# microsoft/crescent-credentials

Measured on AMD Instinct MI355X. Metric: Groth16 proofs/sec (rs256-sd-shaped circuit, BN254), G1 MSM scalar-adds/sec reported alongside, higher is better.
Workload: dtype u32 limbs (BN254 Fq/Fr, 254-bit modular integers)

## Files before the change

crescent-credentials_amd/csrc/msm.hip:

```cpp
#include "msm.hpp"
#include "g2pair.hpp"

#include <chrono>
#include <cstring>
#include <type_traits>

namespace cg {

static constexpr int SCALAR_BITS = 255;

int msm_default_window(uint64_t n, bool precomputed) {
    double best = 1e300;
    int best_c = 4;
    for (int c = 4; c <= 22; ++c) {
        int W = (SCALAR_BITS + c - 1) / c;
        if ((double)W * (double)n >= 2147483648.0) continue;
        double buckets = (double)(1u << (c - 1)) * (precomputed ? 1 : W);
        if (buckets > (double)(1u << 24)) continue;
        double cost = (double)n * W * 12.0 + buckets * 2.0 * 16.0;
        if (cost < best) { best = cost; best_c = c; }
    }
    return best_c;
}

// ... 950 lines not shown
                XYZZ29<F29T> Cu = shfl_up_acc(Cv, d);
                const bool Cuinf = __shfl_up((int)Cinf, d, 64) != 0;
                const bool fu = __shfl_up((int)f, d, 64) != 0;
                if (f) add29(Cv, Cinf, Cu, Cuinf);
                f = f && fu;
            }
        }
        XYZZ29<F29T> Pv = shfl_up_acc(Cv, 1);
        const bool Pinf = __shfl_up((int)Cinf, 1, 64) != 0;
        const unsigned long long chain = __ballot(single && (lane == 0 || joinL));
        auto open_left = [&](unsigned j) { return (~chain & (j >= 63 ? ~0ull : ((2ull << j) - 1ull))) == 0ull; };
        auto emit = [&](uint32_t key, const XYZZ29<F29T>& v, bool vinf, bool touches_left) {
            if (key == NO_KEY) return;
            if (touches_left && !final_level) {
                out_keys[2 * wv] = key;
                store_acc(out_pts + (size_t)(2 * wv) * ACC, v, vinf);
            } else {
                store_acc(bucket_sums + (size_t)key * ACC, v, vinf);
            }
        };
        if (lane > 0 && !joinL) emit(kPrev, Pv, Pinf, open_left(lane - 1));
        if (!single) {
            XYZZ29<F29T> H = A;
            bool Hinf = Ainf, left = lane == 0;
            if (joinL) { add29(H, Hinf, Pv, Pinf); left = open_left(lane - 1); }
            emit(kF, H, Hinf, left);
        }
        if (lane == 63) {
            if (final_level) {
                emit(kL, Cv, Cinf, false);
            } else if (open_left(63)) {
                emit(kL, Cv, Cinf, true);
                out_keys[2 * wv + 1] = kL;
                store_acc(out_pts + (size_t)(2 * wv + 1) * ACC, Cv, true);
            } else {
                out_keys[2 * wv + 1] = kL;
                store_acc(out_pts + (size_t)(2 * wv + 1) * ACC, Cv, Cinf);
            }
        }
    }
}

template <class F29T>
__device__ __forceinline__ void block_tree_sum(XYZZ29<F29T>& acc, bool& inf, uint32_t* sm) {
    constexpr int ACC = Words29<F29T>::ACC;
    store_acc(sm + (size_t)threadIdx.x * ACC, acc, inf);
    __syncthreads();
    for (uint32_t s = blockDim.x / 2; s > 0; s >>= 1) {
        if (threadIdx.x < s) {
            XYZZ29<F29T> b;
            bool bi = load_acc(sm + (size_t)(threadIdx.x + s) * ACC, b);
            add29(acc, inf, b, bi);
            store_acc(sm + (size_t)threadIdx.x * ACC, acc, inf);
        }
        __syncthreads();
    }
}

template <class F29T>
__global__ void __launch_bounds__(256) k_bucket_rows_cols(const uint32_t* __restrict__ buckets, uint32_t R, uint32_t C,
                                                          uint32_t* __restrict__ rows, uint32_t* __restrict__ cols) {
    constexpr int ACC = Words29<F29T>::ACC;
    extern __shared__ __attribute__((aligned(16))) uint32_t sm[];
    const uint32_t w = blockIdx.y, b = blockIdx.x;
    const bool is_row = b < R;
    const uint32_t count = is_row ? C : R, base = is_row ? b * C : b - R, stride = is_row ? 1u : C;
    const uint32_t* src = buckets + (size_t)w * R * C * ACC;
    XYZZ29<F29T> acc;
    bool inf = true;
    for (uint32_t k = threadIdx.x; k < count; k += blockDim.x) {
        XYZZ29<F29T> q;
        bool qinf = load_acc(src + ((size_t)base + (size_t)k * stride) * ACC, q);
        add29(acc, inf, q, qinf);
    }
    block_tree_sum(acc, inf, sm);
    if (threadIdx.x == 0) {
        uint32_t* dst = is_row ? rows + ((size_t)w * R + b) * ACC : cols + ((size_t)w * C + (b - R)) * ACC;
        store_acc(dst, acc, inf);
    }
}

static constexpr uint32_t RED_CHUNK = 32;
template <class F29T>
__global__ void __launch_bounds__(256) k_bucket_chunks(uint32_t* __restrict__ buckets, uint32_t R, uint32_t C,
                                                      uint32_t* __restrict__ rowp, uint32_t* __restrict__ colp, int zero_after) {
    constexpr int ACC = Words29<F29T>::ACC;
    const uint32_t w = blockIdx.y;
    const uint32_t KC = (C + RED_CHUNK - 1) / RED_CHUNK, KR = (R + RED_CHUNK - 1) / RED_CHUNK;
    const uint32_t tile = blockIdx.x * (blockDim.x >> 6) + (threadIdx.x >> 6);
    if (tile >= KR * KC) return;
    const uint32_t tr = tile / KC, tc = tile - tr * KC;
    const uint32_t lane = threadIdx.x & 63u, i = lane & 31u;
    const bool row_lane = lane < 32u;
    uint32_t* src = buckets + (size_t)w * R * C * ACC;
    const uint32_t r0 = tr * RED_CHUNK, c0 = tc * RED_CHUNK;
    const uint32_t nr = R - r0 < RED_CHUNK ? R - r0 : RED_CHUNK, nc = C - c0 < RED_CHUNK ? C - c0 : RED_CHUNK;
    XYZZ29<F29T> acc;
    bool inf = true;
    const bool live = row_lane ? i < nr : i < nc;
    const uint32_t steps = row_lane ? nc : nr;
    for (uint32_t s = 0; s < RED_CHUNK; ++s) {
        if (live && s < steps) {
            const uint32_t r = row_lane ? r0 + i : r0 + s, col = row_lane ? c0 + s : c0 + i;
            XYZZ29<F29T> q;
            bool qinf = load_acc(src + ((size_t)r * C + col) * ACC, q);
            add29(acc, inf, q, qinf);
        }
    }
    if (live) {
        if (row_lane) store_acc(rowp + ((size_t)w * R * KC + (size_t)(r0 + i) * KC + tc) * ACC, acc, inf);
        else store_acc(colp + ((size_t)w * KR * C + (size_t)tr * C + (c0 + i)) * ACC, acc, inf);
    }
    if (zero_after) {
        static_assert(ACC % 4 == 0, "accumulator records are whole uint4s");
        const uint32_t row_vecs = nc * (ACC / 4);
        for (uint32_t r = 0; r < nr; ++r) {
            uint4* dst = reinterpret_cast<uint4*>(src + ((size_t)(r0 + r) * C + c0) * ACC);
            for (uint32_t k = lane; k < row_vecs; k += 64u) dst[k] = make_uint4(0u, 0u, 0u, 0u);
        }
    }
}
template <class F29T>
__global__ void __launch_bounds__(256) k_bucket_chunk_sums(const uint32_t* __restrict__ rowp, const uint32_t* __restrict__ colp, uint32_t R,
                                                          uint32_t C, uint32_t* __restrict__ rows, uint32_t* __restrict__ cols) {
    constexpr int ACC = Words29<F29T>::ACC;
    const uint32_t w = blockIdx.y;
    const uint32_t KC = (C + RED_CHUNK - 1) / RED_CHUNK, KR = (R + RED_CHUNK - 1) / RED_CHUNK;
    const uint32_t n_row = (R + 63u) & ~63u;
    const uint32_t t = blockIdx.x * blockDim.x + threadIdx.x;
    XYZZ29<F29T> acc;
    bool inf = true;
    if (t < n_row) {
        if (t >= R) return;
        const uint32_t* src = rowp + ((size_t)w * R + t) * KC * ACC;
        for (uint32_t k = 0; k < KC; ++k) {
            XYZZ29<F29T> q;
            bool qinf = load_acc(src + (size_t)k * ACC, q);
            add29(acc, inf, q, qinf);
        }
        store_acc(rows + ((size_t)w * R + t) * ACC, acc, inf);
    } else {
        const uint32_t col = t - n_row;
        if (col >= C) return;
        const uint32_t* src = colp + (size_t)w * KR * C * ACC;
        for (uint32_t k = 0; k < KR; ++k) {
            XYZZ29<F29T> q;
            bool qinf = load_acc(src + ((size_t)k * C + col) * ACC, q);
            add29(acc, inf, q, qinf);
        }
        store_acc(cols + ((size_t)w * C + col) * ACC, acc, inf);
    }
}

template <class F29T>
__global__ void __launch_bounds__(256) k_bit_sums(const uint32_t* __restrict__ rows, uint32_t R, uint32_t rbits,
                                                  const uint32_t* __restrict__ cols, uint32_t C, uint32_t* __restrict__ out,
                                                  uint32_t* plan, uint32_t* __restrict__ plan_out, uint32_t zero_words) {
    constexpr int ACC = Words29<F29T>::ACC;
    extern __shared__ __attribute__((aligned(16))) uint32_t sm[];
    const uint32_t w = blockIdx.y, b = blockIdx.x;
    if (w == 0 && b == 0 && threadIdx.x < PLAN_WORDS) {
        plan_out[threadIdx.x] = plan[threadIdx.x];
        if (zero_words) plan[threadIdx.x] = 0;
    }
    if (zero_words) {
        const uint32_t nthr = gridDim.x * gridDim.y * blockDim.x, me = (w * gridDim.x + b) * blockDim.x + threadIdx.x;
        for (uint32_t k = PLAN_WORDS + me; k < zero_words; k += nthr) plan[k] = 0;
    }
    const bool is_row = b < rbits;
    const uint32_t bit = is_row ? b : b - rbits, n = is_row ? R : C, offset = is_row ? 0u : 1u;
    const uint32_t* src = is_row ? rows + (size_t)w * R * ACC : cols + (size_t)w * C * ACC;
    XYZZ29<F29T> acc;
    bool inf = true;
    for (uint32_t i = threadIdx.x; i < n; i += blockDim.x) {
        if (((i + offset) >> bit) & 1u) {
            XYZZ29<F29T> q;
            bool qinf = load_acc(src + (size_t)i * ACC, q);
            add29(acc, inf, q, qinf);
        }
    }
    block_tree_sum(acc, inf, sm);
    if (threadIdx.x == 0) store_acc(out + ((size_t)w * gridDim.x + b) * ACC, acc, inf);
}

static constexpr uint32_t ACC_TARGET_THREADS = 256u * 4u * 4u * 64u;
static constexpr uint32_t G2PAIR_RESIDENT_WAVES = 2;
static constexpr uint32_t ACC_TARGET_PAIRS = 256u * 4u * G2PAIR_RESIDENT_WAVES * 64u / 2u;
template <class F29T> static uint32_t acc_target_segments(bool latency_mode) {
    static const uint32_t quarters = [] { const char* e = CG_TUNE_ENV("ACC_QUARTERS"); const int v = e ? atoi(e) : 4; return (uint32_t)(v >= 1 && v <= 16 ? v : 4); }();
    const uint32_t full = latency_mode ? ACC_TARGET_THREADS : ACC_TARGET_THREADS / 4u * quarters;
    if (Words29<F29T>::NF != 2) return full;
    return g2_pair_kernel(latency_mode) ? ACC_TARGET_PAIRS : full;
}
static constexpr uint32_t ACC_MIN_L = 64, ACC_MIN_L_LATENCY = 16;
static constexpr uint32_t ACC_LEVEL_L = 8;

static int red_cbits(int c) { return (c - 1 + 1) / 2 > 10 ? 10 : (c - 1 + 1) / 2; }

static void part_bits(int c, int W, bool precomputed, int& bits1, int& bits2) {
    int key_bits = c - 1;
    if (!precomputed) key_bits += ilog2_ceil((uint64_t)W);
    if (key_bits < 1) key_bits = 1;
    if (key_bits <= PART_MAX_BITS) { bits1 = key_bits; bits2 = 0; return; }
    bits1 = (key_bits + 1) / 2;
    if (const char* e = CG_TUNE_ENV("PART_BITS1_DELTA")) {
        const int b = bits1 + atoi(e);
        if (b >= 1 && b <= PART_MAX_BITS && key_bits - b >= 1 && key_bits - b <= PART_MAX_BITS) bits1 = b;
    }
    bits2 = key_bits - bits1;
}

template <class F>
void MsmEngine<F>::init(const MsmBases<F>* b, hipStream_t zero_stream) {
    bases = b;
    const uint64_t n = b->n;
    const int W = b->W;
    cap_entries = n * (uint64_t)W;
    if (cap_entries == 0) cap_entries = 1;
    const uint32_t nb = 1u << (b->c - 1);
    nbuckets_total = b->precomputed ? nb : nb * (uint32_t)W;
    part_bits(b->c, W, b->precomputed, bits1, bits2);
    if (bits1 > PART_MAX_BITS || bits2 > PART_MAX_BITS) throw HipError(CG_ERR_INVALID_ARGUMENT, "bucket key space too large");
    const uint32_t B1 = 1u << bits1;
    const uint64_t tiles = n ? ceil_div(n, PART_TILE) : 1;
    blk_hist.alloc(tiles * B1);
    const size_t keyspace = bits2 ? ((size_t)1 << (bits1 + bits2)) : 0;
    counters.alloc(PLAN_WORDS + 2 * (size_t)B1 * PART_PAD + 2 * keyspace);
    starts.alloc(2 * ((size_t)B1 + 1) + 2);
    max_chunks = bits2 ? (uint32_t)(cap_entries / PART_CHUNK) + B1 + 1 : 0;
    bucket_sums.alloc(((size_t)nbuckets_total + 1) * ACC);
    min_L = latency_mode ? ACC_MIN_L_LATENCY : ACC_MIN_L;
    if (const char* e = CG_TUNE_ENV("MIN_SEGMENT")) {
        const int v = atoi(e);
        if (v >= 1 && v <= 4096) min_L = (uint32_t)v;
    }
    uint64_t t1 = (cap_entries + min_L - 1) / min_L;
    if (t1 > acc_target_segments<F29T>(latency_mode)) t1 = acc_target_segments<F29T>(latency_mode);
    max_segments = (uint32_t)t1;
    uint64_t pa = 2 * t1, pb = 0;
    for (uint64_t w = ceil_div(t1, 64); ; w = ceil_div(w, 64)) { pb += 2 * w; if (w <= 1) break; }
    mem().reserve(cap_entries, bits2 ? cap_entries : 1, pa, pa * ACC, pb, pb * ACC);
    const uint32_t wins = b->precomputed ? 1u : (uint32_t)W;
    {
        const int cbits = red_cbits(b->c);
        const uint32_t C = 1u << cbits, R = nb / C;
        red_rbits = ilog2_ceil((uint64_t)R);
        red_cbits1 = cbits + 1;
        rows_buf.alloc((size_t)R * wins * ACC);
        cols_buf.alloc((size_t)C * wins * ACC);
        if (!latency_mode) {
            rowp_buf.alloc((size_t)R * ceil_div(C, RED_CHUNK) * wins * ACC);
            colp_buf.alloc((size_t)ceil_div(R, RED_CHUNK) * C * wins * ACC);
        }
    }
    if (zero_stream) {
        CG_HIP(hipMemsetAsync(counters.p, 0, counters.bytes(), zero_stream));
        CG_HIP(hipMemsetAsync(bucket_sums.p, 0, bucket_sums.bytes(), zero_stream));
    } else {
        hipStream_t zs = nullptr;
        CG_HIP(hipStreamCreateWithFlags(&zs, hipStreamNonBlocking));
        hipError_t e1 = hipMemsetAsync(counters.p, 0, counters.bytes(), zs);
        hipError_t e2 = hipMemsetAsync(bucket_sums.p, 0, bucket_sums.bytes(), zs);
        hipError_t e3 = hipStreamSynchronize(zs);
        (void)hipStreamDestroy(zs);
        CG_HIP(e1); CG_HIP(e2); CG_HIP(e3);
// ... 8 lines not shown

template <class F>
void MsmEngine<F>::device_bytes(uint64_t& entries, uint64_t& pieces, uint64_t& other) const {
    entries += own_mem.entry_bytes();
    pieces += own_mem.piece_bytes();
    other += blk_hist.bytes() + counters.bytes() + starts.bytes() + bucket_sums.bytes() + rows_buf.bytes() + cols_buf.bytes() +
             rowp_buf.bytes() + colp_buf.bytes();
}

static float elapsed_ms(hipEvent_t a, hipEvent_t b) {
    float ms = 0;
    if (hipEventElapsedTime(&ms, a, b) != hipSuccess) return 0.f;
    return ms;
}
template <class F> float MsmEngine<F>::ms_total() const { return elapsed_ms(ev_t[0], ev_t[5]); }
template <class F> float MsmEngine<F>::ms_sort() const { return n_scalars ? elapsed_ms(ev_t[1], ev_t[2]) : 0.f; }
template <class F> float MsmEngine<F>::ms_accum() const { return n_scalars ? elapsed_ms(ev_t[3], ev_t[4]) : 0.f; }

template <class F>
MsmEngine<F>::~MsmEngine() {
    for (auto& e : ev_t) if (e) (void)hipEventDestroy(e);
}

template <class F>
void MsmEngine<F>::digits(const Fr* scalars_dev, uint64_t n, hipStream_t st) {
    if (n > bases->n) n = bases->n;
    n_scalars = n;
    adopted = nullptr;
    for (int k = 0; k < PLAN_WORDS; ++k) h_plan.p[k] = 0;
    CG_HIP(hipEventRecord(ev_t[0], st));
    if (!n) {
        if (!counters_clean) fill_zero(counters.p, (counters.bytes() + 15) & ~(size_t)15, st);
        counters_clean = zero_at_end;
        return;
    }
    const uint32_t B1 = 1u << bits1;
    uint32_t* plan = counters.p;
    uint32_t* hist1 = plan + PLAN_WORDS;
    uint32_t* cur1 = hist1 + (size_t)B1 * PART_PAD;
    uint32_t* hist2 = cur1 + (size_t)B1 * PART_PAD;
    uint32_t* cur2 = hist2 + (bits2 ? ((size_t)1 << (bits1 + bits2)) : 0);
    uint32_t* start1 = starts.p;
    uint32_t* chunk0 = starts.p + B1 + 1;
    PartShape sh;
    sh.n = (uint32_t)n; sh.c = bases->c; sh.W = bases->W; sh.precomputed = bases->precomputed ? 1 : 0;
    sh.row_stride = (uint32_t)bases->n;
    sh.bits1 = bits1; sh.bits2 = bits2;
    sh.staged = latency_mode ? 1 : 0;
    const uint32_t tiles = ceil_div(n, PART_TILE);
    CG_HIP(hipEventRecord(ev_t[1], st));
    if (!counters_clean) fill_zero(counters.p, (counters.bytes() + 15) & ~(size_t)15, st);
    counters_clean = false;
    PlanArgs pa;
    pa.start1 = start1; pa.chunk0 = chunk0; pa.target_threads = acc_target_segments<F29T>(latency_mode); pa.min_L = min_L;
    pa.two_level = bits2 ? 1 : 0;
    launch_part_level1(true, sh, tiles, (size_t)B1 * 4, st, scalars_dev, bases->valid.p, blk_hist.p, hist1, plan, nullptr, nullptr, nullptr, pa);
    CG_KERNEL_CHECK();
    launch_part_level1(false, sh, tiles, (size_t)B1 * 4, st, scalars_dev, bases->valid.p, blk_hist.p, nullptr, nullptr, start1, cur1, mem().ent_a.p, pa);
    CG_KERNEL_CHECK();
    if (bits2) {
        const uint32_t B2 = 1u << bits2;
        k_part_count2<<<max_chunks, 256, (size_t)B2 * 4, st>>>(bits1, bits2, mem().ent_a.p, chunk0, start1, hist2);
        CG_KERNEL_CHECK();
        k_part_place2<<<max_chunks, 256, (size_t)B2 * 16 + (size_t)PART_CHUNK * 8, st>>>(bits1, bits2, mem().ent_a.p, chunk0, start1, hist2, cur2, mem().ent_b.p);
        CG_KERNEL_CHECK();
    }
    CG_HIP(hipEventRecord(ev_t[2], st));
}

template <class F>
void MsmEngine<F>::adopt(const uint64_t* grouped_entries, const uint32_t* plan_dev, uint64_t n, hipStream_t st) {
    if (n > bases->n) n = bases->n;
    n_scalars = n;
    for (int k = 0; k < PLAN_WORDS; ++k) h_plan.p[k] = 0;
    CG_HIP(hipEventRecord(ev_t[0], st));
    CG_HIP(hipEventRecord(ev_t[1], st));
    k_replan<<<1, 1, 0, st>>>(counters.p, plan_dev, acc_target_segments<F29T>(latency_mode), min_L);
    counters_clean = false;
    CG_KERNEL_CHECK();
    CG_HIP(hipEventRecord(ev_t[2], st));
    adopted = n ? grouped_entries : nullptr;
}

template <class F>
void MsmEngine<F>::accumulate(hipStream_t st) {
    if (!buckets_clean) fill_zero(bucket_sums.p, bucket_sums.bytes(), st);
    buckets_clean = false;
    if (n_scalars) {
        const uint32_t* plan = counters.p;
        const uint64_t* grouped = adopted ? adopted : this->grouped();
        CG_HIP(hipEventRecord(ev_t[3], st));
        static const bool knock_accum = CG_TUNE_ENV("KNOCK_ACCUM") != nullptr, knock_combine = CG_TUNE_ENV("KNOCK_COMBINE") != nullptr;
        if (!knock_accum)
            launch_accum_affine<F29T>(grouped, plan, max_segments, bases->table.p, bucket_sums.p, mem().part_keys_a.p, mem().part_pts_a.p, latency_mode, st);
        CG_KERNEL_CHECK();
        CG_HIP(hipEventRecord(ev_t[4], st));
        if (max_segments > 1 && !knock_accum && !knock_combine) {
            MsmScratch& S = mem();
            uint32_t segs = max_segments;
            for (int level = 0; segs > 1; ++level) {
                const uint32_t waves = ceil_div(segs, 64u);
                k_combine_wave<F29T><<<ceil_div(waves, tail_block<F29T>() / 64u), tail_block<F29T>(), 0, st>>>(S.part_keys_a.p, S.part_pts_a.p, plan, bucket_sums.p, S.part_keys_b.p, S.part_pts_b.p, level);
                CG_KERNEL_CHECK();
                segs = waves;
            }
        }
    }
    enqueue_reduction(st);
    CG_HIP(hipEventRecord(ev_t[5], st));
}

template <class F>
void MsmEngine<F>::enqueue_reduction(hipStream_t st) {
    const uint32_t wins = bases->precomputed ? 1u : (uint32_t)bases->W;
    const uint32_t nb = 1u << (bases->c - 1);
    const uint32_t C = 1u << red_cbits(bases->c), R = nb / C;
    const size_t lds = (size_t)256 * ACC * 4;
    static const bool force_tree = CG_TUNE_ENV("RED_TREE") != nullptr;
    static const bool knock_tail = CG_TUNE_ENV("KNOCK_TAIL") != nullptr;
    if (knock_tail) return;
    if (latency_mode || force_tree) {
        k_bucket_rows_cols<F29T><<<dim3(R + C, wins), 256, lds, st>>>(bucket_sums.p, R, C, rows_buf.p, cols_buf.p);
        CG_KERNEL_CHECK();
    } else {
        const uint32_t KC = ceil_div(C, RED_CHUNK), KR = ceil_div(R, RED_CHUNK);
        const uint32_t lanes_b = ((R + 63u) & ~63u) + C;
        const uint32_t tb = tail_block<F29T>();
        k_bucket_chunks<F29T><<<dim3(ceil_div(KR * KC, tb / 64u), wins), tb, 0, st>>>(bucket_sums.p, R, C, rowp_buf.p, colp_buf.p, zero_at_end ? 1 : 0);
        CG_KERNEL_CHECK();
        buckets_clean = zero_at_end;
        k_bucket_chunk_sums<F29T><<<dim3(ceil_div(lanes_b, tb), wins), tb, 0, st>>>(rowp_buf.p, colp_buf.p, R, C, rows_buf.p, cols_buf.p);
        CG_KERNEL_CHECK();
    }
    const uint32_t nbits = (uint32_t)(red_rbits + red_cbits1);
    k_bit_sums<F29T><<<dim3(nbits, wins), 256, lds, st>>>(rows_buf.p, R, (uint32_t)red_rbits, cols_buf.p, C, h_result.dev(), counters.p,
                                                          h_plan.dev(), zero_at_end ? (uint32_t)counters.n : 0u);
    CG_KERNEL_CHECK();
    counters_clean = zero_at_end;
}

static Fq fq_from_limbs29(const uint32_t l[9]) {
    typedef unsigned __int128 u128;
    uint64_t v[5] = {0, 0, 0, 0, 0};
    for (int i = 0; i < 9; ++i) {
        int bit = 29 * i, w = bit >> 6, sh = bit & 63;
        u128 x = (u128)l[i] << sh;
        u128 s = (u128)v[w] + (uint64_t)x;
        v[w] = (uint64_t)s;
        u128 carry = (s >> 64) + (x >> 64);
        for (int k = w + 1; k < 5 && carry; ++k) {
            u128 t = (u128)v[k] + (uint64_t)carry;
            v[k] = (uint64_t)t;
            carry = t >> 64;
        }
    }
    uint64_t n[5] = {0, 0, 0, 0, 0};
    for (int i = 0; i < 4; ++i) n[i] = (uint64_t)FqP::N[2 * i] | ((uint64_t)FqP::N[2 * i + 1] << 32);
    auto ge = [&]() {
        for (int i = 4; i >= 0; --i) {
            if (v[i] > n[i]) return true;
            if (v[i] < n[i]) return false;
        }
        return true;
    };
    while (ge()) {
        u128 br = 0;
        for (int i = 0; i < 5; ++i) {
            u128 d = (u128)v[i] - n[i] - (uint64_t)br;
            v[i] = (uint64_t)d;
            br = (d >> 64) & 1;
        }
    }
    Fq a;
    for (int i = 0; i < 4; ++i) { a.l[2 * i] = (uint32_t)v[i]; a.l[2 * i + 1] = (uint32_t)(v[i] >> 32); }
    Fq c2 = Fq::zero();
    c2.l[7] = 0x08000000u;
    return mul(a, c2);
}
static void coord_from_limbs29(Fq& out, const uint32_t* w) { out = fq_from_limbs29(w); }
static void coord_from_limbs29(Fq2& out, const uint32_t* w) { out.c0 = fq_from_limbs29(w); out.c1 = fq_from_limbs29(w + 9); }

template <class F>
static XYZZ<F> xyzz_from_words(const uint32_t* w, int acc_words) {
    const int q = acc_words / 4;
    bool inf = true;
    for (int i = 0; i < q; ++i) if (w[2 * q + i]) inf = false;
    if (inf) return XYZZ<F>::inf();
    XYZZ<F> r;
    coord_from_limbs29(r.x, w);
    coord_from_limbs29(r.y, w + q);
    coord_from_limbs29(r.zz, w + 2 * q);
    coord_from_limbs29(r.zzz, w + 3 * q);
    return r;
}

template <class F>
static XYZZ<F> fold_bits(const uint32_t* bit_sums, int n, int acc_words) {
    XYZZ<F> acc = XYZZ<F>::inf();
    for (int k = n - 1; k >= 0; --k) {
        acc = dbl(acc);
        add(acc, xyzz_from_words<F>(bit_sums + (size_t)k * acc_words, acc_words));
    }
    return acc;
}
template <class F>
static XYZZ<F> window_value(const uint32_t* bit_sums, int acc_words, int rbits, int cbits1) {
    XYZZ<F> rows = fold_bits<F>(bit_sums, rbits, acc_words);
    XYZZ<F> cols = fold_bits<F>(bit_sums + (size_t)rbits * acc_words, cbits1, acc_words);
    for (int k = 0; k < cbits1 - 1; ++k) rows = dbl(rows);
    add(rows, cols);
    return rows;
}

template <class F>
XYZZ<F> MsmEngine<F>::value() const {
    const int nbits = red_rbits + red_cbits1;
    if (bases->precomputed) return window_value<F>(h_result.p, ACC, red_rbits, red_cbits1);
    const int W = bases->W, c = bases->c;
    XYZZ<F> acc = XYZZ<F>::inf();
    for (int j = W - 1; j >= 0; --j) {
        for (int k = 0; k < c; ++k) acc = dbl(acc);
// ... 115 lines not shown
```

crescent-credentials_amd/csrc/msm.hpp:

```cpp
#pragma once
#include "common.hpp"
#include "curve29.hpp"
#include "ntt.hpp"

#include <functional>

namespace cg {

template <class F>
struct MsmBases {
    typedef typename To29<F>::type F29T;
    static constexpr int AFF = Words29<F29T>::AFF;
    uint64_t n = 0;
    int c = 0;
    int W = 0;
    bool precomputed = true;
    DevBuf<uint32_t> table;
    DevBuf<uint8_t> valid;
    void build(const Affine<F>* bases_dev, uint64_t n, int c, bool precompute, hipStream_t st);
    void build_from_row0(const uint32_t* row0_dev, const uint8_t* valid_dev, uint64_t n, int c, hipStream_t st);
    int rebuild(int c_new, hipStream_t st);
    void alloc_rows(uint64_t n, int c, bool precompute);
    void expand_rows(hipStream_t st);
};

int msm_default_window(uint64_t n, bool precomputed);
int msm_best_window(uint64_t n_bases, double nz_small, double nz_full);

struct MsmScratch {
    DevBuf<uint64_t> ent_a, ent_b;
    DevBuf<uint32_t> part_keys_a, part_keys_b;
    DevBuf<uint32_t> part_pts_a, part_pts_b;
    uint64_t entry_bytes() const { return ent_a.bytes() + ent_b.bytes(); }
    uint64_t piece_bytes() const { return part_keys_a.bytes() + part_keys_b.bytes() + part_pts_a.bytes() + part_pts_b.bytes(); }
    void reserve(size_t n_ent_a, size_t n_ent_b, size_t keys_a, size_t pts_a, size_t keys_b, size_t pts_b) {
        if (ent_a.n < n_ent_a) ent_a.alloc(n_ent_a);
        if (ent_b.n < n_ent_b) ent_b.alloc(n_ent_b);
        if (part_keys_a.n < keys_a) part_keys_a.alloc(keys_a);
        if (part_pts_a.n < pts_a) part_pts_a.alloc(pts_a);
        if (part_keys_b.n < keys_b) part_keys_b.alloc(keys_b);
        if (part_pts_b.n < pts_b) part_pts_b.alloc(pts_b);
    }
};

template <class F>
struct MsmEngine {
    typedef typename To29<F>::type F29T;
    static constexpr int ACC = Words29<F29T>::ACC;
    const MsmBases<F>* bases = nullptr;
    uint64_t cap_entries = 0;
    uint32_t nbuckets_total = 0;
    MsmScratch own_mem;
    MsmScratch* shared_mem = nullptr;
    MsmScratch& mem() { return shared_mem ? *shared_mem : own_mem; }
    const MsmScratch& mem() const { return shared_mem ? *shared_mem : own_mem; }
    int bits1 = 0, bits2 = 0;
    DevBuf<uint32_t> blk_hist;
    DevBuf<uint32_t> counters;
    DevBuf<uint32_t> starts;
    uint32_t max_chunks = 0;
    uint32_t min_L = 16;
    uint32_t max_segments = 0;
    DevBuf<uint32_t> bucket_sums;
    DevBuf<uint32_t> rows_buf, cols_buf;
    DevBuf<uint32_t> rowp_buf, colp_buf;
    int red_rbits = 0, red_cbits1 = 0;
    PinnedBuf<uint32_t> h_plan;
    PinnedBuf<uint32_t> h_result;
    uint64_t n_scalars = 0;
    bool zero_at_end = false;
    bool counters_clean = false, buckets_clean = false;
    bool latency_mode = false;
    uint32_t n_entries() const { return h_plan.p ? h_plan.p[0] : 0; }
    uint32_t n_nonzero() const { return h_plan.p ? h_plan.p[3] : 0; }
    void enqueue_reduction(hipStream_t st);
    hipEvent_t ev_t[6] = {nullptr, nullptr, nullptr, nullptr, nullptr, nullptr};
    float ms_total() const;
    float ms_sort() const;
    float ms_accum() const;

    void init(const MsmBases<F>* b, hipStream_t zero_stream = nullptr);
    ~MsmEngine();
    void device_bytes(uint64_t& entries, uint64_t& pieces, uint64_t& other) const;
    void digits(const Fr* scalars_dev, uint64_t n, hipStream_t st);
    template <class G>
    bool can_adopt(const MsmEngine<G>& src) const {
        return bases->precomputed && src.bases->precomputed && bases->n == src.bases->n && bases->c == src.bases->c &&
               bits1 == src.bits1 && bits2 == src.bits2;
    }
    void adopt(const uint64_t* grouped_entries, const uint32_t* plan_dev, uint64_t n, hipStream_t st);
    const uint64_t* grouped() const { return bits2 ? mem().ent_b.p : mem().ent_a.p; }
    const uint64_t* adopted = nullptr;
    void accumulate(hipStream_t st);
    XYZZ<F> value() const;
};

void ec_inverse_dft(const uint32_t* row0_in, const uint8_t* valid_in, uint64_t n_in, int logn, const Fr& scale_base,
                    const Fr& scale_mult, uint32_t* row0_out, uint8_t* valid_out, hipStream_t st);
void ec_transform_h_bases(const uint32_t* row0_in, const uint8_t* valid_in, uint64_t n_in, int logn, uint32_t* row0_out,
                          uint8_t* valid_out, hipStream_t st);
void ec_fold_c_into_l(const uint32_t* h_row0, const uint8_t* h_valid, uint64_t n_h, int logn, const Fr& vanishing_inv,
                      const cg_csr& c_matrix, uint64_t num_constraints, uint64_t num_inputs, uint64_t M,
                      const uint32_t* l_row0, const uint8_t* l_valid, uint32_t* row0_out, uint8_t* valid_out, hipStream_t st);
void ec_fold_ct_into_l(const uint32_t* h_row0, const uint8_t* h_valid, uint64_t n_h, int logn, const Fr& vanishing_inv,
                       const HostCsc& c_transposed, uint64_t num_constraints, uint64_t num_inputs, uint64_t M,
                       const uint32_t* l_row0, const uint8_t* l_valid, uint32_t* row0_out, uint8_t* valid_out, hipStream_t st);
void sum_xyzz_by_key(const uint32_t* keys, const uint32_t* pts, uint64_t count, uint32_t* sums, hipStream_t st);
void build_hl_bases_folded(MsmBases<Fq>& out_h, MsmBases<Fq>& out_l, const Affine<Fq>* h_bases_dev, uint64_t n_h, int logn,
                           const Affine<Fq>* l_bases_dev, uint64_t num_inputs, uint64_t M, const cg_csr& c_matrix,
                           uint64_t num_constraints, const Fr& vanishing_inv, uint64_t h_first, uint64_t h_stride, uint64_t h_count,
                           int c_h, uint64_t l_first, uint64_t l_count, int c_l, hipStream_t st, float* ms_fold = nullptr,
                           float* ms_tables = nullptr);

void build_h_bases_folded(MsmBases<Fq>& out_h, const uint32_t* h_row0, const uint8_t* h_valid, uint64_t n_h, int logn, uint64_t h_first,
                          uint64_t h_stride, uint64_t h_count, int c_h, hipStream_t st, float* ms_fold, float* ms_tables);
void build_l_bases_folded(MsmBases<Fq>& out_l, const uint32_t* h_row0, const uint8_t* h_valid, uint64_t n_h, int logn,
                          const uint32_t* l_row0, const uint8_t* l_valid, uint64_t num_inputs, uint64_t M, const HostCsc& c_transposed,
                          uint64_t num_constraints, const Fr& vanishing_inv, uint64_t l_first, uint64_t l_count,
                          const std::function<int()>& pick_c_l, hipStream_t st, float* ms_fold, float* ms_tables);

template <class F>
void import_bases(const uint8_t* host_bytes, uint32_t coord_form, uint64_t n, Affine<F>* out_dev, hipStream_t st);

extern template struct MsmBases<Fq>;
extern template struct MsmBases<Fq2>;
extern template struct MsmEngine<Fq>;
extern template struct MsmEngine<Fq2>;

}
```

crescent-credentials_amd/csrc/prover.hip:

```cpp
#include <atomic>
#include <condition_variable>
#include <shared_mutex>
#include <memory>
#include <mutex>
#include <chrono>
#include <cstdlib>
#include <exception>
#include <functional>
#include <thread>

#include "msm.hpp"
#include "ntt.hpp"
#include "wmap29.hpp"

namespace cg {

const char* csr_view_problem(const cg_csr& m);

std::string& last_error() {
    static thread_local std::string e;
    return e;
}
int fail(int code, const char* fmt, ...) {
    char buf[1024];
// ... 919 lines not shown
    for (int i = 0; i < 5; ++i)
        if (i == 0 || S->st[i] != S->st[0]) CG_HIP(hipEventSynchronize(S->ev_fin[i]));
}

static float upload_assignment(cg_ctx* c, Upload* u, const void* host_assignment, bool timed) {
    if (timed) CG_HIP(hipEventRecord(u->ev[0], u->st));
    CG_HIP(hipMemcpyAsync(u->w.p, host_assignment, c->M * 32, hipMemcpyHostToDevice, u->st));
    if (timed) CG_HIP(hipEventRecord(u->ev[1], u->st));
    if (c->spin_wait || c->latency) {
        CG_HIP(hipStreamSynchronize(u->st));
    } else {
        CG_HIP(hipEventRecord(u->ev_done, u->st));
        wait_sleeping(u->ev_done, 50);
    }
    return timed ? ev_ms(u->ev[0], u->ev[1]) : 0.f;
}

static const char* const BROKEN_CONTEXT = "a window re-tune ran out of device memory while re-sizing the proof slots: free this context and load the circuit again";

struct CallFrame {
    CallGuard inside;
    cg_ctx* const c;
    const Fr* w_dev = nullptr;
    ProofSlot* S = nullptr;
    float upload_ms = 0.f;
    CallFrame(cg_ctx* ctx, const void* assignment, bool on_device, bool may_run_alone, bool timed = false, bool handle = false)
        : inside(ctx), c(ctx), in_handle(handle), exceptions(std::uncaught_exceptions()) {
        try {
            if (c->broken) throw HipError(CG_ERR_OUT_OF_MEMORY, BROKEN_CONTEXT);
            CG_HIP(hipSetDevice(c->device));
            if (in_handle) c->tune_mu.lock_shared_passing_waiting_writers();
            else c->tune_mu.lock_shared();
            gate_held = true;
            if (c->broken) throw HipError(CG_ERR_OUT_OF_MEMORY, BROKEN_CONTEXT);
            w_dev = (const Fr*)assignment;
            if (!on_device) {
                up = c->acquire_upload();
                upload_ms = upload_assignment(c, up, assignment, timed);
                w_dev = up->w.p;
            }
            S = c->acquire(may_run_alone);
        } catch (...) {
            release();
            throw;
        }
    }
    ~CallFrame() { release(); }
    void release() {
        if (S) {
            if (in_handle || std::uncaught_exceptions() > exceptions)
                for (auto st : S->st) if (st) (void)hipStreamSynchronize(st);
            c->release(S);
            S = nullptr;
        }
        if (up) {
            (void)hipStreamSynchronize(up->st);
            c->release_upload(up);
            up = nullptr;
        }
        if (gate_held) { c->tune_mu.unlock_shared(); gate_held = false; }
    }
private:
    Upload* up = nullptr;
    bool gate_held = false;
    const bool in_handle;
    const int exceptions;
};

static bool no_share_b() {
    static const bool v = CG_TUNE_ENV("NO_SHARE_B") != nullptr;
    return v;
}
static int knock_mask() {
    static const int v = [] { const char* e = CG_TUNE_ENV("KNOCK"); return e ? atoi(e) : 0; }();
    return v;
}

struct Schedule {
    ProofSlot* const S;
    const Fr *w_l, *w_a;
    uint64_t n_l, n_a;
    bool run_l, run_a, run_b1, run_b2;
    bool b2_adopts;
    Schedule(const cg_ctx* c, ProofSlot* slot, const Fr* w_dev, bool skip_b1) : S(slot) {
        w_l = w_dev + (c->folded ? 0 : c->l) + c->rl.lo;
        w_a = w_dev + 1 + c->ra.lo;
        n_l = c->rl.hi - c->rl.lo;
        n_a = c->ra.hi - c->ra.lo;
        const int knock = knock_mask();
        run_l = !(knock & 1); run_a = !(knock & 2); run_b1 = !skip_b1 && !(knock & 4); run_b2 = !(knock & 8);
        b2_adopts = run_b1 && run_b2 && !no_share_b() && c->b_same_identities && S->eb2.can_adopt(S->eb1) && n_a > 0;
    }
    void phase1() const {
        hipStream_t s0 = S->st[0];
        if (S->one_stream) {
            if (run_l) { S->el.digits(w_l, n_l, s0); S->el.accumulate(s0); }
            if (run_a) { S->ea.digits(w_a, n_a, s0); S->ea.accumulate(s0); }
            if (run_b1) S->eb1.digits(w_a, n_a, s0);
            if (b2_adopts) S->eb2.adopt(S->eb1.grouped(), S->eb1.counters.p, n_a, s0);
            if (run_b1) S->eb1.accumulate(s0);
            if (run_b2 && !b2_adopts) S->eb2.digits(w_a, n_a, s0);
            if (run_b2) S->eb2.accumulate(s0);
            return;
        }
        CG_HIP(hipEventRecord(S->ev_w, s0));
        for (int i = 1; i < 5; ++i) CG_HIP(hipStreamWaitEvent(S->st[i], S->ev_w, 0));
        if (run_l) S->el.digits(w_l, n_l, S->st[1]);
        if (run_a) S->ea.digits(w_a, n_a, S->st[2]);
        if (run_b1) S->eb1.digits(w_a, n_a, S->st[3]);
        if (b2_adopts) {
            CG_HIP(hipEventRecord(S->ev_b1, S->st[3]));
            CG_HIP(hipStreamWaitEvent(S->st[4], S->ev_b1, 0));
            S->eb2.adopt(S->eb1.grouped(), S->eb1.counters.p, n_a, S->st[4]);
        } else if (run_b2) {
            S->eb2.digits(w_a, n_a, S->st[4]);
        }
    }
    void phase2() const {
        if (S->one_stream) return;
        if (run_l) S->el.accumulate(S->st[1]);
        if (run_a) S->ea.accumulate(S->st[2]);
        if (run_b1) S->eb1.accumulate(S->st[3]);
        if (run_b2) S->eb2.accumulate(S->st[4]);
    }
};

static void snapshot_tune_stats(const cg_ctx* c, const ProofSlot* S, bool skip_b1, TuneStats& ts);

static int collect(cg_ctx* c, ProofSlot* S, bool skip_b1, bool h_supplied, bool in_one_call, std::chrono::steady_clock::time_point t0,
                   Partials& P, cg_timings* tm, TuneStats& ts) {
    wait_for_slot(c, S);
    if (int e = input_verdict(c, S, h_supplied, c->check_witness && !h_supplied)) return e;
    P.h = to_affine(S->eh.value());
    P.l = to_affine(S->el.value());
    P.a = to_affine(S->ea.value());
    P.b1 = skip_b1 ? G1Affine::inf() : to_affine(S->eb1.value());
    P.b2 = to_affine(S->eb2.value());
    if (knock_mask() && tm) { memset(tm, 0, sizeof(*tm)); tm = nullptr; }
    if (tm) {
        memset(tm, 0, sizeof(*tm));
        tm->msm_h_ms = S->eh.ms_total();
        tm->msm_l_ms = S->el.ms_total();
        tm->msm_a_ms = S->ea.ms_total();
        tm->msm_b1_ms = skip_b1 ? 0.f : S->eb1.ms_total();
        tm->msm_b2_ms = S->eb2.ms_total();
        if (in_one_call) {
            tm->witness_map_ms = ev_ms(S->ev_t[0], S->ev_t[1]);
            tm->accum_g1_ms = S->eh.ms_accum() + S->el.ms_accum() + S->ea.ms_accum() + (skip_b1 ? 0.f : S->eb1.ms_accum());
            tm->accum_g2_ms = S->eb2.ms_accum();
            tm->sort_ms = S->eh.ms_sort() + S->el.ms_sort() + S->ea.ms_sort() + (skip_b1 ? 0.f : S->eb1.ms_sort()) + S->eb2.ms_sort();
            tm->entries_g1 = (uint64_t)S->eh.n_entries() + S->el.n_entries() + S->ea.n_entries() + (skip_b1 ? 0 : S->eb1.n_entries());
            tm->entries_g2 = S->eb2.n_entries();
            tm->accum_g1_launches = (S->eh.n_entries() != 0) + (S->el.n_entries() != 0) + (S->ea.n_entries() != 0) + (!skip_b1 && S->eb1.n_entries() != 0);
            tm->accum_g2_launches = S->eb2.n_entries() != 0;
            tm->msm_g1_pairs = S->eh.n_scalars + S->el.n_scalars + S->ea.n_scalars + (skip_b1 ? 0 : S->eb1.n_scalars);
            tm->msm_g2_pairs = S->eb2.n_scalars;
        }
        tm->total_ms = ms_since(t0);
    }
    snapshot_tune_stats(c, S, skip_b1, ts);
    return CG_OK;
}

static int prove_partial_impl(cg_ctx* c, ProofSlot* S, const Fr* w_dev, bool skip_b1, Partials& P, cg_timings* tm, TuneStats& ts,
                              const std::function<void()>* while_gpu_runs = nullptr, const SuppliedH* supplied = nullptr) {
    const auto t0 = std::chrono::steady_clock::now();
    hipStream_t s0 = S->st[0];
    const Schedule sch(c, S, w_dev, skip_b1);
    const int knock = knock_mask();
    sch.phase1();
    if (tm) CG_HIP(hipEventRecord(S->ev_t[0], s0));
    const Fr* h_scalars = (knock & 16) && S->knock_h ? S->knock_h : witness_map_or_check(c, S, w_dev, supplied);
    if (knock & 16) S->knock_h = h_scalars;
    if (tm) CG_HIP(hipEventRecord(S->ev_t[1], s0));
    if (!(knock & 32)) S->eh.digits(h_scalars, c->rh.hi - c->rh.lo, s0);
    sch.phase2();
    if (!(knock & 32)) S->eh.accumulate(s0);
    if (while_gpu_runs) (*while_gpu_runs)();
    return collect(c, S, !sch.run_b1, supplied != nullptr, true, t0, P, tm, ts);
}

struct DeltaMultiples {
    G1XYZZ r_g1, rs_delta, s_g1;
    G2XYZZ s_g2;
};
static DeltaMultiples delta_multiples(const cg_ctx* c, const uint8_t r[32], const uint8_t s[32]) {
    DeltaMultiples d;
    d.r_g1 = c->fb_delta_g1.mul(r);
    uint8_t rs[32];
    fp_to_bytes(from_mont(mul(to_mont(fp_from_bytes<Fr>(r)), to_mont(fp_from_bytes<Fr>(s)))), rs);
    d.rs_delta = c->fb_delta_g1.mul(rs);
    d.s_g1 = c->fb_delta_g1.mul(s);
    d.s_g2 = c->fb_delta_g2.mul(s);
    return d;
}

static void assemble_impl(const cg_ctx* c, const Partials& S, const uint8_t r[32], const uint8_t s[32], uint8_t proof_out[256],
                          const DeltaMultiples* pre = nullptr) {
    const bool r_zero = scalar_is_zero(r);
    DeltaMultiples local;
    if (!pre) { local = delta_multiples(c, r, s); pre = &local; }
    const G1XYZZ& r_g1 = pre->r_g1;
    const G1XYZZ& rs_delta = pre->rs_delta;
    G1XYZZ g_a = r_g1;
    madd(g_a, c->a0);
    madd(g_a, S.a);
    madd(g_a, c->alpha_g1);
    G1XYZZ s_g_a = scalar_mul_bytes(g_a, s);
    G1XYZZ g1_b = G1XYZZ::inf();
    if (!r_zero) {
        g1_b = pre->s_g1;
        madd(g1_b, c->b1_0);
        madd(g1_b, S.b1);
        madd(g1_b, c->beta_g1);
    }
    G2XYZZ g2_b = pre->s_g2;
    madd(g2_b, c->b2_0);
    madd(g2_b, S.b2);
    madd(g2_b, c->beta_g2);
    G1XYZZ r_g1_b = scalar_mul_bytes(g1_b, r);
    G1XYZZ g_c = s_g_a;
    add(g_c, r_g1_b);
    add(g_c, neg(rs_delta));
    madd(g_c, S.l);
    madd(g_c, S.h);
    g1_serialize_uncompressed(to_affine(g_a), proof_out);
    g2_serialize_uncompressed(to_affine(g2_b), proof_out + 64);
    g1_serialize_uncompressed(to_affine(g_c), proof_out + 192);
}

static void partials_to_bytes(const Partials& P, uint8_t out[384]) {
    g1_export_canonical(P.h, out);
    g1_export_canonical(P.l, out + 64);
    g1_export_canonical(P.a, out + 128);
    g1_export_canonical(P.b1, out + 192);
    g2_export_canonical(P.b2, out + 256);
}

static constexpr int RETUNE_MAX_ATTEMPTS = 8;
template <class F>
static TuneStats::Q tune_stats_of(const MsmEngine<F>& e) {
    TuneStats::Q q;
    q.n_scalars = e.n_scalars; q.nonzero = e.n_nonzero(); q.entries = e.n_entries(); q.W0 = e.bases->W;
    return q;
}
static void snapshot_tune_stats(const cg_ctx* c, const ProofSlot* S, bool skip_b1, TuneStats& ts) {
    if (c->fixed_window || c->tuned || c->retune_attempts >= RETUNE_MAX_ATTEMPTS) return;
    ts.l = tune_stats_of(S->el); ts.a = tune_stats_of(S->ea); ts.b2 = tune_stats_of(S->eb2);
    if (!skip_b1) ts.b1 = tune_stats_of(S->eb1);
    ts.valid = true;
}
template <class F>
static void reinit_engines(cg_ctx* c, MsmEngine<F> ProofSlot::*eng, const MsmBases<F>& bases) {
    try {
        if (const char* f = CG_TUNE_ENV("FAULT_RETUNE")) if (f[0] == '1') throw HipError(CG_ERR_OUT_OF_MEMORY, "injected: out of device memory while re-sizing the proof slots");
        for (size_t k = 0; k < c->slots.size(); ++k) ((*c->slots[k]).*eng).init(&bases);
    } catch (...) {
        c->broken = true;
        throw;
    }
// ... 385 lines not shown
```

Baseline: 169.4.

## Batch deferred G1 MSM bucket reductions into shared multi-job kernel launches

When all MSMs run on a single stream with one shard, the bucket-reduction tails of the L, A, B1 and H G1 engines are deferred and then issued together. Each of the three reduction kernels (chunk partials, chunk sums, bit sums) is launched once with a job table that maps each block to its engine. This replaces four small launches per stage with one larger grid, cutting launch overhead and filling the GPU better on tail kernels. The cost is a block-to-job lookup inside each kernel, and the batched path only covers precomputed, non-latency engines.

After: 175.9, median of 6. +3.8%, better.

```diff
diff --git a/crescent-credentials_amd/csrc/msm.hip b/crescent-credentials_amd/csrc/msm.hip
--- a/crescent-credentials_amd/csrc/msm.hip
+++ b/crescent-credentials_amd/csrc/msm.hip
@@ -1056,12 +1056,11 @@
 
 static constexpr uint32_t RED_CHUNK = 32;
 template <class F29T>
-__global__ void __launch_bounds__(256) k_bucket_chunks(uint32_t* __restrict__ buckets, uint32_t R, uint32_t C,
-                                                      uint32_t* __restrict__ rowp, uint32_t* __restrict__ colp, int zero_after) {
+__device__ __forceinline__ void bucket_chunks_block(const uint32_t bx, const uint32_t w, uint32_t* __restrict__ buckets, uint32_t R, uint32_t C,
+                                                    uint32_t* __restrict__ rowp, uint32_t* __restrict__ colp, int zero_after) {
     constexpr int ACC = Words29<F29T>::ACC;
-    const uint32_t w = blockIdx.y;
     const uint32_t KC = (C + RED_CHUNK - 1) / RED_CHUNK, KR = (R + RED_CHUNK - 1) / RED_CHUNK;
-    const uint32_t tile = blockIdx.x * (blockDim.x >> 6) + (threadIdx.x >> 6);
+    const uint32_t tile = bx * (blockDim.x >> 6) + (threadIdx.x >> 6);
     if (tile >= KR * KC) return;
     const uint32_t tr = tile / KC, tc = tile - tr * KC;
     const uint32_t lane = threadIdx.x & 63u, i = lane & 31u;
@@ -1095,13 +1094,18 @@
     }
 }
 template <class F29T>
-__global__ void __launch_bounds__(256) k_bucket_chunk_sums(const uint32_t* __restrict__ rowp, const uint32_t* __restrict__ colp, uint32_t R,
-                                                          uint32_t C, uint32_t* __restrict__ rows, uint32_t* __restrict__ cols) {
+__global__ void __launch_bounds__(256) k_bucket_chunks(uint32_t* __restrict__ buckets, uint32_t R, uint32_t C,
+                                                      uint32_t* __restrict__ rowp, uint32_t* __restrict__ colp, int zero_after) {
+    bucket_chunks_block<F29T>(blockIdx.x, blockIdx.y, buckets, R, C, rowp, colp, zero_after);
+}
+template <class F29T>
+__device__ __forceinline__ void bucket_chunk_sums_block(const uint32_t bx, const uint32_t w, const uint32_t* __restrict__ rowp,
+                                                        const uint32_t* __restrict__ colp, uint32_t R, uint32_t C,
+                                                        uint32_t* __restrict__ rows, uint32_t* __restrict__ cols) {
     constexpr int ACC = Words29<F29T>::ACC;
-    const uint32_t w = blockIdx.y;
     const uint32_t KC = (C + RED_CHUNK - 1) / RED_CHUNK, KR = (R + RED_CHUNK - 1) / RED_CHUNK;
     const uint32_t n_row = (R + 63u) & ~63u;
-    const uint32_t t = blockIdx.x * blockDim.x + threadIdx.x;
+    const uint32_t t = bx * blockDim.x + threadIdx.x;
     XYZZ29<F29T> acc;
     bool inf = true;
     if (t < n_row) {
@@ -1125,20 +1129,25 @@
         store_acc(cols + ((size_t)w * C + col) * ACC, acc, inf);
     }
 }
-
-template <class F29T>
-__global__ void __launch_bounds__(256) k_bit_sums(const uint32_t* __restrict__ rows, uint32_t R, uint32_t rbits,
-                                                  const uint32_t* __restrict__ cols, uint32_t C, uint32_t* __restrict__ out,
-                                                  uint32_t* plan, uint32_t* __restrict__ plan_out, uint32_t zero_words) {
+template <class F29T>
+__global__ void __launch_bounds__(256) k_bucket_chunk_sums(const uint32_t* __restrict__ rowp, const uint32_t* __restrict__ colp, uint32_t R,
+                                                          uint32_t C, uint32_t* __restrict__ rows, uint32_t* __restrict__ cols) {
+    bucket_chunk_sums_block<F29T>(blockIdx.x, blockIdx.y, rowp, colp, R, C, rows, cols);
+}
+
+template <class F29T>
+__device__ __forceinline__ void bit_sums_block(const uint32_t b, const uint32_t w, const uint32_t nbits, const uint32_t wins,
+                                               const uint32_t* __restrict__ rows, uint32_t R, uint32_t rbits,
+                                               const uint32_t* __restrict__ cols, uint32_t C, uint32_t* __restrict__ out,
+                                               uint32_t* plan, uint32_t* __restrict__ plan_out, uint32_t zero_words) {
     constexpr int ACC = Words29<F29T>::ACC;
     extern __shared__ __attribute__((aligned(16))) uint32_t sm[];
-    const uint32_t w = blockIdx.y, b = blockIdx.x;
     if (w == 0 && b == 0 && threadIdx.x < PLAN_WORDS) {
         plan_out[threadIdx.x] = plan[threadIdx.x];
         if (zero_words) plan[threadIdx.x] = 0;
     }
     if (zero_words) {
-        const uint32_t nthr = gridDim.x * gridDim.y * blockDim.x, me = (w * gridDim.x + b) * blockDim.x + threadIdx.x;
+        const uint32_t nthr = nbits * wins * blockDim.x, me = (w * nbits + b) * blockDim.x + threadIdx.x;
         for (uint32_t k = PLAN_WORDS + me; k < zero_words; k += nthr) plan[k] = 0;
     }
     const bool is_row = b < rbits;
@@ -1154,7 +1163,50 @@
         }
     }
     block_tree_sum(acc, inf, sm);
-    if (threadIdx.x == 0) store_acc(out + ((size_t)w * gridDim.x + b) * ACC, acc, inf);
+    if (threadIdx.x == 0) store_acc(out + ((size_t)w * nbits + b) * ACC, acc, inf);
+}
+template <class F29T>
+__global__ void __launch_bounds__(256) k_bit_sums(const uint32_t* __restrict__ rows, uint32_t R, uint32_t rbits,
+                                                  const uint32_t* __restrict__ cols, uint32_t C, uint32_t* __restrict__ out,
+                                                  uint32_t* plan, uint32_t* __restrict__ plan_out, uint32_t zero_words) {
+    bit_sums_block<F29T>(blockIdx.x, blockIdx.y, gridDim.x, gridDim.y, rows, R, rbits, cols, C, out, plan, plan_out, zero_words);
+}
+
+static constexpr int RED_BATCH_MAX = 4;
+struct RedJob {
+    uint32_t *buckets, *rowp, *colp, *rows, *cols;
+    uint32_t *out, *plan, *plan_out;
+    uint32_t R, C, rbits, cbits1;
+    uint32_t zero_words;
+};
+struct RedBatch {
+    RedJob job[RED_BATCH_MAX];
+    uint32_t end[RED_BATCH_MAX];
+    uint32_t n;
+};
+__device__ __forceinline__ uint32_t red_batch_job(const RedBatch& B, uint32_t& bx) {
+    uint32_t j = 0;
+    bx = blockIdx.x;
+    while (j + 1 < B.n && blockIdx.x >= B.end[j]) bx = blockIdx.x - B.end[j++];
+    return j;
+}
+template <class F29T>
+__global__ void __launch_bounds__(256) k_bucket_chunks_batch(const RedBatch B) {
+    uint32_t bx;
+    const RedJob& J = B.job[red_batch_job(B, bx)];
+    bucket_chunks_block<F29T>(bx, 0u, J.buckets, J.R, J.C, J.rowp, J.colp, J.zero_words ? 1 : 0);
+}
+template <class F29T>
+__global__ void __launch_bounds__(256) k_bucket_chunk_sums_batch(const RedBatch B) {
+    uint32_t bx;
+    const RedJob& J = B.job[red_batch_job(B, bx)];
+    bucket_chunk_sums_block<F29T>(bx, 0u, J.rowp, J.colp, J.R, J.C, J.rows, J.cols);
+}
+template <class F29T>
+__global__ void __launch_bounds__(256) k_bit_sums_batch(const RedBatch B) {
+    uint32_t bx;
+    const RedJob& J = B.job[red_batch_job(B, bx)];
+    bit_sums_block<F29T>(bx, 0u, J.rbits + J.cbits1, 1u, J.rows, J.R, J.rbits, J.cols, J.C, J.out, J.plan, J.plan_out, J.zero_words);
 }
 
 static constexpr uint32_t ACC_TARGET_THREADS = 256u * 4u * 4u * 64u;
@@ -1329,8 +1381,14 @@
     adopted = n ? grouped_entries : nullptr;
 }
 
-template <class F>
-void MsmEngine<F>::accumulate(hipStream_t st) {
+static bool red_force_tree() {
+    static const bool v = CG_TUNE_ENV("RED_TREE") != nullptr;
+    return v;
+}
+
+template <class F>
+void MsmEngine<F>::accumulate(hipStream_t st, bool defer_reduction) {
+    reduction_pending = false;
     if (!buckets_clean) fill_zero(bucket_sums.p, bucket_sums.bytes(), st);
     buckets_clean = false;
     if (n_scalars) {
@@ -1353,7 +1411,8 @@
             }
         }
     }
-    enqueue_reduction(st);
+    if (defer_reduction && n_scalars && bases->precomputed && !latency_mode && !red_force_tree()) reduction_pending = true;
+    else enqueue_reduction(st);
     CG_HIP(hipEventRecord(ev_t[5], st));
 }
 
@@ -1363,7 +1422,7 @@
     const uint32_t nb = 1u << (bases->c - 1);
     const uint32_t C = 1u << red_cbits(bases->c), R = nb / C;
     const size_t lds = (size_t)256 * ACC * 4;
-    static const bool force_tree = CG_TUNE_ENV("RED_TREE") != nullptr;
+    const bool force_tree = red_force_tree();
     static const bool knock_tail = CG_TUNE_ENV("KNOCK_TAIL") != nullptr;
     if (knock_tail) return;
     if (latency_mode || force_tree) {
@@ -1384,6 +1443,53 @@
                                                           h_plan.dev(), zero_at_end ? (uint32_t)counters.n : 0u);
     CG_KERNEL_CHECK();
     counters_clean = zero_at_end;
+}
+
+void enqueue_reduction_batch(MsmEngine<Fq>* const* engines, int n, hipStream_t st) {
+    typedef MsmEngine<Fq>::F29T F29T;
+    constexpr int ACC = MsmEngine<Fq>::ACC;
+    static const bool knock_tail = CG_TUNE_ENV("KNOCK_TAIL") != nullptr;
+    const uint32_t tb = tail_block<F29T>();
+    RedBatch chunks, sums, bits;
+    MsmEngine<Fq>* in[RED_BATCH_MAX];
+    uint32_t m = 0;
+    for (int k = 0; k < n; ++k) {
+        MsmEngine<Fq>* e = engines[k];
+        if (!e || !e->reduction_pending) continue;
+        e->reduction_pending = false;
+        if (knock_tail) continue;
+        if (m == RED_BATCH_MAX) throw HipError(CG_ERR_INVALID_ARGUMENT, "more bucket sets than one reduction batch holds");
+        const uint32_t nb = 1u << (e->bases->c - 1);
+        RedJob J;
+        J.C = 1u << red_cbits(e->bases->c); J.R = nb / J.C;
+        J.rbits = (uint32_t)e->red_rbits; J.cbits1 = (uint32_t)e->red_cbits1;
+        J.buckets = e->bucket_sums.p; J.rowp = e->rowp_buf.p; J.colp = e->colp_buf.p; J.rows = e->rows_buf.p; J.cols = e->cols_buf.p;
+        J.out = e->h_result.dev(); J.plan = e->counters.p; J.plan_out = e->h_plan.dev();
+        J.zero_words = e->zero_at_end ? (uint32_t)e->counters.n : 0u;
+        const uint32_t KC = ceil_div(J.C, RED_CHUNK), KR = ceil_div(J.R, RED_CHUNK);
+        const uint32_t lanes_b = ((J.R + 63u) & ~63u) + J.C;
+        const uint32_t e0 = m ? chunks.end[m - 1] : 0u, e1 = m ? sums.end[m - 1] : 0u, e2 = m ? bits.end[m - 1] : 0u;
+        chunks.job[m] = sums.job[m] = bits.job[m] = J;
+        chunks.end[m] = e0 + ceil_div(KR * KC, tb / 64u);
+        sums.end[m] = e1 + ceil_div(lanes_b, tb);
+        bits.end[m] = e2 + J.rbits + J.cbits1;
+        in[m++] = e;
+    }
+    if (!m) return;
+    for (uint32_t k = m; k < RED_BATCH_MAX; ++k) {
+        chunks.job[k] = sums.job[k] = bits.job[k] = chunks.job[0];
+        chunks.end[k] = chunks.end[m - 1]; sums.end[k] = sums.end[m - 1]; bits.end[k] = bits.end[m - 1];
+    }
+    chunks.n = sums.n = bits.n = m;
+    k_bucket_chunks_batch<F29T><<<chunks.end[m - 1], tb, 0, st>>>(chunks);
+    CG_KERNEL_CHECK();
+    for (uint32_t k = 0; k < m; ++k) in[k]->buckets_clean = in[k]->zero_at_end;
+    k_bucket_chunk_sums_batch<F29T><<<sums.end[m - 1], tb, 0, st>>>(sums);
+    CG_KERNEL_CHECK();
+    k_bit_sums_batch<F29T><<<bits.end[m - 1], 256, (size_t)256 * ACC * 4, st>>>(bits);
+    CG_KERNEL_CHECK();
+    for (uint32_t k = 0; k < m; ++k) in[k]->counters_clean = in[k]->zero_at_end;
+    CG_HIP(hipEventRecord(in[m - 1]->ev_t[5], st));
 }
 
 static Fq fq_from_limbs29(const uint32_t l[9]) {
diff --git a/crescent-credentials_amd/csrc/msm.hpp b/crescent-credentials_amd/csrc/msm.hpp
--- a/crescent-credentials_amd/csrc/msm.hpp
+++ b/crescent-credentials_amd/csrc/msm.hpp
@@ -74,6 +74,7 @@
     uint32_t n_entries() const { return h_plan.p ? h_plan.p[0] : 0; }
     uint32_t n_nonzero() const { return h_plan.p ? h_plan.p[3] : 0; }
     void enqueue_reduction(hipStream_t st);
+    bool reduction_pending = false;
     hipEvent_t ev_t[6] = {nullptr, nullptr, nullptr, nullptr, nullptr, nullptr};
     float ms_total() const;
     float ms_sort() const;
@@ -91,9 +92,11 @@
     void adopt(const uint64_t* grouped_entries, const uint32_t* plan_dev, uint64_t n, hipStream_t st);
     const uint64_t* grouped() const { return bits2 ? mem().ent_b.p : mem().ent_a.p; }
     const uint64_t* adopted = nullptr;
-    void accumulate(hipStream_t st);
+    void accumulate(hipStream_t st, bool defer_reduction = false);
     XYZZ<F> value() const;
 };
+
+void enqueue_reduction_batch(MsmEngine<Fq>* const* engines, int n, hipStream_t st);
 
 void ec_inverse_dft(const uint32_t* row0_in, const uint8_t* valid_in, uint64_t n_in, int logn, const Fr& scale_base,
                     const Fr& scale_mult, uint32_t* row0_out, uint8_t* valid_out, hipStream_t st);
diff --git a/crescent-credentials_amd/csrc/prover.hip b/crescent-credentials_amd/csrc/prover.hip
--- a/crescent-credentials_amd/csrc/prover.hip
+++ b/crescent-credentials_amd/csrc/prover.hip
@@ -1025,7 +1025,9 @@
     uint64_t n_l, n_a;
     bool run_l, run_a, run_b1, run_b2;
     bool b2_adopts;
+    bool defer;
     Schedule(const cg_ctx* c, ProofSlot* slot, const Fr* w_dev, bool skip_b1) : S(slot) {
+        defer = S->one_stream && c->shard_count == 1;
         w_l = w_dev + (c->folded ? 0 : c->l) + c->rl.lo;
         w_a = w_dev + 1 + c->ra.lo;
         n_l = c->rl.hi - c->rl.lo;
@@ -1037,11 +1039,11 @@
     void phase1() const {
         hipStream_t s0 = S->st[0];
         if (S->one_stream) {
-            if (run_l) { S->el.digits(w_l, n_l, s0); S->el.accumulate(s0); }
-            if (run_a) { S->ea.digits(w_a, n_a, s0); S->ea.accumulate(s0); }
+            if (run_l) { S->el.digits(w_l, n_l, s0); S->el.accumulate(s0, defer); }
+            if (run_a) { S->ea.digits(w_a, n_a, s0); S->ea.accumulate(s0, defer); }
             if (run_b1) S->eb1.digits(w_a, n_a, s0);
             if (b2_adopts) S->eb2.adopt(S->eb1.grouped(), S->eb1.counters.p, n_a, s0);
-            if (run_b1) S->eb1.accumulate(s0);
+            if (run_b1) S->eb1.accumulate(s0, defer);
             if (run_b2 && !b2_adopts) S->eb2.digits(w_a, n_a, s0);
             if (run_b2) S->eb2.accumulate(s0);
             return;
@@ -1065,6 +1067,11 @@
         if (run_a) S->ea.accumulate(S->st[2]);
         if (run_b1) S->eb1.accumulate(S->st[3]);
         if (run_b2) S->eb2.accumulate(S->st[4]);
+    }
+    void tails(bool run_h) const {
+        if (!defer) return;
+        MsmEngine<Fq>* const g1[4] = {run_l ? &S->el : nullptr, run_a ? &S->ea : nullptr, run_b1 ? &S->eb1 : nullptr, run_h ? &S->eh : nullptr};
+        enqueue_reduction_batch(g1, 4, S->st[0]);
     }
 };
 
@@ -1118,7 +1125,8 @@
     if (tm) CG_HIP(hipEventRecord(S->ev_t[1], s0));
     if (!(knock & 32)) S->eh.digits(h_scalars, c->rh.hi - c->rh.lo, s0);
     sch.phase2();
-    if (!(knock & 32)) S->eh.accumulate(s0);
+    if (!(knock & 32)) S->eh.accumulate(s0, sch.defer);
+    sch.tails(!(knock & 32));
     if (while_gpu_runs) (*while_gpu_runs)();
     return collect(c, S, !sch.run_b1, supplied != nullptr, true, t0, P, tm, ts);
 }
```
